# cockroachdb/pebble

Hardware: AMD Instinct MI355X
Metric: raw-block GiB/s decoded to KV arrays (device-resident), 1/2/4/8 MI355X (higher is better)
Workload: dtype u8; 1 GPU; config2: 65536 x 32 KiB row-format blocks per GPU, restart interval 16, 16 B keys / 100 B values; blocks_per_gpu=65536, input_bytes_per_gpu=2143748096, kvs_per_gpu=17760256, global_batch_blocks=65536, parallelism=shard1

## Files before the change

pebble_amd/csrc/rowblk_big.hip.h:

```cpp
#pragma once

#include "rowblk_core.hip.h"
#include "rowblk_general.hip.h"

namespace pbl {
namespace row {
namespace rowc {

#ifndef PBL_BIG_WIN
#define PBL_BIG_WIN 8
#endif
#ifndef PBL_BIG_U
#define PBL_BIG_U 8
#endif
#ifndef PBL_BIG_KEYBUF
#define PBL_BIG_KEYBUF 8192
#endif
constexpr uint32_t kBigKeySmall = PBL_BIG_KEYBUF;
constexpr int kWsBigRedo = 5;
constexpr int kWsBigPend = 6;
constexpr int kWsBigLong = 7;

__device__ __forceinline__ void big_block_publish(const Args& A, uint32_t b, const SlowState& ss) {
  const uint32_t nb = A.in.n_blocks;
  uint64_t* lb_state = reinterpret_cast<uint64_t*>(reinterpret_cast<uint8_t*>(A.out.workspace) + kWsHeader);
  const bool okk = ss.status == PBL_OK;
  const uint64_t agg[kNumComp] = {okk ? ss.nkv : 0, okk ? ss.kb : 0, okk ? ss.vb : 0, okk ? ss.nr : 0};
  lb_publish(lb_state, nb, b, agg);
  if (lane_id() == 0) {
    to_glb(A.out.blk_status)[b] = ss.status;
    to_glb(A.out.blk_kv_base)[b] = agg[0];
    to_glb(A.out.blk_key_base)[b] = agg[1];
    to_glb(A.out.blk_val_base)[b] = agg[2];
  }
}

template <bool kSpill = false>
__device__ __forceinline__ void big_block_count(const Args& A, uint32_t b, lptr<uint8_t> keybuf, uint32_t keycap,
                                                SlowState* ss, gptr<uint8_t> spill = nullptr, uint64_t spillcap = 0) {
  const uint32_t blen = A.in.block_len[b];
  const uint8_t* gblk = A.in.blocks + A.in.block_off[b];
  uint32_t roff, nres;
  const uint32_t st = init_checks(GlbBlk{to_glb(gblk), blen}, blen, A.in.flags, &roff, &nres);
  if (st != PBL_OK) {
    ss->nkv = ss->kb = ss->vb = ss->nr = 0;
    ss->status = st;
    return;
  }
  const uint64_t dummy[kNumComp] = {0, 0, 0, 0};
  slow_walk_t<GlbBlk, 1, kSpill>(GlbBlk{to_glb(gblk), blen}, blen, A.in.flags, A.in.synthetic_seq_num, keybuf, keycap,
                                  kPassCount, A.out, b, dummy, ss, spill, spillcap);
}

__global__ void __launch_bounds__(kWave) big_block_sizes_kernel(Args A) {
  __shared__ uint4 keybuf4[kBigKeySmall / 16];
  const uint32_t nb = A.in.n_blocks;
  uint32_t* hdr = reinterpret_cast<uint32_t*>(A.out.workspace);
  uint32_t* redo = reinterpret_cast<uint32_t*>(reinterpret_cast<uint8_t*>(A.out.workspace) + ws_redo_offset(nb));
  for (uint64_t base = uint64_t(blockIdx.x) * PBL_BIG_WIN; base < nb; base += uint64_t(gridDim.x) * PBL_BIG_WIN) {
    const uint64_t bl = base + lane_id();
    uint64_t big = __ballot(lane_id() < PBL_BIG_WIN && bl < nb && to_glb(A.in.block_len)[bl] > kMaxFastLen &&
                            (!A.in.block_format || to_glb(A.in.block_format)[bl] == PBL_FMT_ROW));
    while (big) {
      const uint32_t b = uint32_t(base) + uint32_t(__builtin_ctzll(big));
      big &= big - 1;
      SlowState ss;
      big_block_count(A, b, to_lds_ptr(reinterpret_cast<uint8_t*>(keybuf4)), kBigKeySmall, &ss);
      if (ss.status == PBL_UNSUPPORTED) {
        if (lane_id() == 0) to_glb(redo)[g_atomic_add(hdr + kWsBigRedo, 1u)] = b;
        continue;
      }
      big_block_publish(A, b, ss);
    }
  }
}

template <bool kList>
__device__ __forceinline__ void big_block_sizes2_body(const Args& A, uint4* keybuf4) {
  const uint32_t nb = A.in.n_blocks;
  const uint32_t* hdr = reinterpret_cast<const uint32_t*>(A.out.workspace);
  const uint32_t n = __hip_atomic_load(to_glb(hdr) + kWsBigRedo, __ATOMIC_RELAXED, __HIP_MEMORY_SCOPE_AGENT);
  const uint32_t* redo = reinterpret_cast<const uint32_t*>(reinterpret_cast<uint8_t*>(A.out.workspace) +
                                                           ws_redo_offset(nb));
  for (uint32_t i = blockIdx.x; i < n; i += gridDim.x) {
    const uint32_t b = to_glb(redo)[i];
    SlowState ss;
    big_block_count(A, b, to_lds_ptr(reinterpret_cast<uint8_t*>(keybuf4)), uint32_t(kLdsBlkBytes), &ss);
    if constexpr (kList) {
      if (ss.status == PBL_UNSUPPORTED && !((ss.kb | ss.vb) >> 32)) {
        uint32_t* lng = reinterpret_cast<uint32_t*>(reinterpret_cast<uint8_t*>(A.out.workspace) + ws_ent_offset(nb));
        if (lane_id() == 0) to_glb(lng)[g_atomic_add(const_cast<uint32_t*>(hdr) + kWsBigLong, 1u)] = b;
        continue;
      }
    }
    big_block_publish(A, b, ss);
  }
}

__global__ void __launch_bounds__(kWave) big_block_sizes2_kernel(Args A) {
  __shared__ uint4 keybuf4[kLdsBlkBytes / 16];
  big_block_sizes2_body<false>(A, keybuf4);
}

__global__ void __launch_bounds__(kWave) big_block_values_kernel(Args A) {
  __shared__ uint4 keybuf4[kLdsBlkBytes / 16];
  const uint32_t nb = A.in.n_blocks;
  const uint32_t* hdr = reinterpret_cast<const uint32_t*>(A.out.workspace);
  const uint32_t n = __hip_atomic_load(to_glb(hdr) + kWsBigPend, __ATOMIC_RELAXED, __HIP_MEMORY_SCOPE_AGENT);
  const uint32_t* pend = reinterpret_cast<const uint32_t*>(reinterpret_cast<const uint8_t*>(A.out.workspace) +
                                                           ws_pend_offset(nb));
  for (uint32_t i = blockIdx.x; i < n; i += gridDim.x) {
    const uint32_t b = to_glb(pend)[i];
    const uint32_t blen = A.in.block_len[b];
    const uint64_t bases[kNumComp] = {A.out.blk_kv_base[b], A.out.blk_key_base[b], A.out.blk_val_base[b],
                                      A.out.blk_rst_base ? A.out.blk_rst_base[b] : 0};
    SlowState ss;
    slow_walk_t<GlbBlk, PBL_BIG_U>(GlbBlk{to_glb(A.in.blocks + A.in.block_off[b]), blen}, blen, A.in.flags,
                                    A.in.synthetic_seq_num, to_lds_ptr(reinterpret_cast<uint8_t*>(keybuf4)),
                                    uint32_t(kLdsBlkBytes), kPassAll, A.out, b, bases, &ss);
  }
}

}
}
}
```

pebble_amd/csrc/rowblk_decode.hip:

```cpp
#include <algorithm>
#include <atomic>

#include "common.hip.h"
#include "colblk_block.hip.h"
#include "rowblk_core.hip.h"
#include "rowblk_general.hip.h"
#include "rowblk_big.hip.h"
#include "rowblk_pool.hip.h"
#include "rowblk_wave.hip.h"

#define PBL_COL_PIPE_BODY_ONLY
#include "colblk_pipe.hip.h"
#include "colblk_wave.hip.h"

namespace pbl {
namespace row {


__global__ void __launch_bounds__(kTPB) mixed_split_count_kernel(Args A, uint32_t* counts) {
  const uint32_t nb = A.in.n_blocks;
  const uint32_t c0 = blockIdx.x * kSplitChunk;
  uint32_t k = 0;
  for (uint32_t i = c0 + threadIdx.x; i < nb && i < c0 + kSplitChunk; i += kTPB)
    k += to_glb(A.in.block_format)[i] == PBL_FMT_ROW;
// ... 107 lines not shown
    kvb[i] += d[0];
    kb[i] += d[1];
    vb[i] += d[2];
    if (rb) rb[i] += d[3];
  }
}

}
}

namespace pbl {

namespace {
constexpr int kMaxDevices = 64;
std::atomic<int> g_cus[kMaxDevices];
std::atomic<int> g_per_cu[kMaxDevices][kKNum];
}

uint64_t persistent_grid(hipStream_t st, PersistentKernel k, const void* fn, uint64_t n_units, int* cus_out,
                         int block_threads) {
  int dev = -1;
  if (st ? hipStreamGetDevice(st, &dev) != hipSuccess : hipGetDevice(&dev) != hipSuccess) return 0;
  if (dev < 0 || dev >= kMaxDevices) return 0;
  int cus = g_cus[dev].load(std::memory_order_relaxed);
  int per_cu = g_per_cu[dev][k].load(std::memory_order_relaxed);
  if (cus <= 0 || per_cu <= 0) {
    int cur = -1;
    if (hipGetDevice(&cur) != hipSuccess) return 0;
    if (cur != dev && hipSetDevice(dev) != hipSuccess) return 0;
    const bool ok = hipDeviceGetAttribute(&cus, hipDeviceAttributeMultiprocessorCount, dev) == hipSuccess &&
                    hipOccupancyMaxActiveBlocksPerMultiprocessor(&per_cu, fn, block_threads, 0) == hipSuccess;
    if (cur != dev) (void)hipSetDevice(cur);
    if (!ok) return 0;
    cus = cus > 0 ? cus : 1;
    per_cu = per_cu > 0 ? per_cu : 1;
    g_cus[dev].store(cus, std::memory_order_relaxed);
    g_per_cu[dev][k].store(per_cu, std::memory_order_relaxed);
  }
  if (cus_out) *cus_out = cus;
  uint64_t grid = uint64_t(cus) * uint64_t(per_cu);
  if (grid > n_units) grid = n_units;
  return grid ? grid : 1;
}

}

#include "rowblk_long.hip.h"

namespace {
bool has_spill_slots(const pbl::Args& a) {
  return pbl::ws_spill_slot_bytes(a.out.workspace_bytes, a.in.n_blocks) != 0;
}

void launch_big_sizes(const pbl::Args& a, hipStream_t st, uint32_t small) {
  const uint32_t g1 = (a.in.n_blocks + PBL_BIG_WIN - 1) / PBL_BIG_WIN;
  hipLaunchKernelGGL(pbl::row::rowc::big_block_sizes_kernel, dim3(g1), dim3(pbl::kWave), 0, st, a);
  if (!has_spill_slots(a)) {
    hipLaunchKernelGGL(pbl::row::rowc::big_block_sizes2_kernel, dim3(small), dim3(pbl::kWave), 0, st, a);
    return;
  }
  hipLaunchKernelGGL(pbl::row::rowc::long_key_sizes2_kernel, dim3(small), dim3(pbl::kWave), 0, st, a);
  hipLaunchKernelGGL(pbl::row::rowc::long_key_sizes_kernel, dim3(pbl::kLongKeyWgs), dim3(pbl::kWave), 0, st, a);
}

void launch_long_values(const pbl::Args& a, hipStream_t st, uint64_t list_off, int count_word) {
  if (has_spill_slots(a))
    hipLaunchKernelGGL(pbl::row::rowc::long_key_values_kernel, dim3(pbl::kLongKeyWgs), dim3(pbl::kWave), 0, st, a,
                       list_off, count_word);
}

void launch_big_values(const pbl::Args& a, hipStream_t st, uint32_t small) {
  hipLaunchKernelGGL(pbl::row::rowc::big_block_values_kernel, dim3(small), dim3(pbl::kWave), 0, st, a);
  launch_long_values(a, st, pbl::ws_ent_offset(a.in.n_blocks), pbl::row::rowc::kWsBigLong);
}

uint64_t pool_grid(hipStream_t st, bool hide, uint32_t nb, int* cus) {
  namespace pool = pbl::row::pool;
  const void* fn = pbl::with_bool(
      hide, [](auto h) { return reinterpret_cast<const void*>(pool::rowblk_pool_kernel<decltype(h)::value>); });
  return pbl::persistent_grid(st, pbl::kKRowPool, fn, (uint64_t(nb) + pool::kNW - 1) / pool::kNW, cus, pool::kTPBP);
}

void launch_pool(const pbl::Args& a, hipStream_t st, bool hide, uint64_t grid, const uint32_t* ids) {
  namespace pool = pbl::row::pool;
  pbl::with_bool(hide, [&](auto h) {
    hipLaunchKernelGGL(pool::rowblk_pool_kernel<decltype(h)::value>, dim3(uint32_t(grid)), dim3(pool::kTPBP), 0, st, a,
                       ids);
  });
}

int launch_row_pool(const pbl::Args& a, hipStream_t st, bool values) {
  const uint32_t nb = a.in.n_blocks;
  const bool hide = (a.in.flags & PBL_ROW_HIDE_OBSOLETE) && !(a.in.flags & PBL_ROW_RAW_KEYS);
  int cus = 0;
  const uint64_t grid = pool_grid(st, hide, nb, &cus);
  if (!grid) return PBL_DEVICE_ERROR;
  const uint32_t small = uint32_t(std::min<uint64_t>(nb, uint64_t(cus > 0 ? cus : 1) * 4));
  launch_big_sizes(a, st, small);
  launch_pool(a, st, hide, grid, nullptr);
  if (values) launch_big_values(a, st, small);
  return hipGetLastError() == hipSuccess ? PBL_OK : PBL_DEVICE_ERROR;
}

int launch_mixed(const pbl_block_batch* batch, const pbl::Args& a, hipStream_t st, bool values) {
  const bool hide = (batch->flags & PBL_ROW_HIDE_OBSOLETE) != 0;
  const bool hide_rows = hide && !(batch->flags & PBL_ROW_RAW_KEYS);
  const uint32_t nb = batch->n_blocks;
  uint8_t* ws = reinterpret_cast<uint8_t*>(a.out.workspace);
  uint32_t* ids = reinterpret_cast<uint32_t*>(ws + pbl::ws_ids_offset(nb));
  uint32_t* counts = ids + nb;
  const uint32_t nch = (nb + pbl::kSplitChunk - 1) / pbl::kSplitChunk;
  hipLaunchKernelGGL(pbl::row::mixed_split_count_kernel, dim3(nch), dim3(pbl::kTPB), 0, st, a, counts);
  hipLaunchKernelGGL(pbl::row::mixed_split_scatter_kernel, dim3(nch), dim3(pbl::kTPB), 0, st, a,
                     static_cast<const uint32_t*>(counts), nch, ids);
  int cus = 0;
  const void* cfn = pbl::with_bool(
      hide, [](auto h) { return reinterpret_cast<const void*>(pbl::row::mixed_col_kernel<decltype(h)::value>); });
  const uint64_t g_c = pbl::persistent_grid(st, hide ? pbl::kKMixedColHide : pbl::kKMixedCol, cfn, nb, &cus);
  if (!g_c) return PBL_DEVICE_ERROR;
  const uint32_t small = uint32_t(std::min<uint64_t>(nb, uint64_t(cus > 0 ? cus : 1) * 4));
  const uint32_t* cids = static_cast<const uint32_t*>(ids);
  launch_big_sizes(a, st, small);
  const uint32_t g_cs = uint32_t(std::min<uint64_t>(nb, uint64_t(cus > 0 ? cus : 1) * 4 * PBL_CW_SWAVES));
  pbl::with_bool(hide, [&](auto h) {
    hipLaunchKernelGGL((pbl::col::cwave::colblk_wave_size_kernel<true, decltype(h)::value>), dim3(g_cs),
                       dim3(pbl::kWave), 0, st, a, cids);
  });
  const uint64_t g_p = pool_grid(st, hide_rows, nb, &cus);
  if (!g_p) return PBL_DEVICE_ERROR;
  launch_pool(a, st, hide_rows, g_p, cids);
#ifndef PBL_MIX_COL_WAVE
#define PBL_MIX_COL_WAVE 1
#endif
  if (!hide && PBL_MIX_COL_WAVE)
    hipLaunchKernelGGL((pbl::col::cwave::colblk_wave_emit_kernel<PBL_CW_STAGE, true>), dim3(nb), dim3(pbl::kWave), 0,
                       st, a, cids);
  else
    pbl::with_bool(hide, [&](auto h) {
      hipLaunchKernelGGL(pbl::row::mixed_col_kernel<decltype(h)::value>, dim3(uint32_t(g_c)), dim3(pbl::kTPB), 0, st,
                         a, cids);
    });
  if (values) launch_big_values(a, st, small);
  return hipGetLastError() == hipSuccess ? PBL_OK : PBL_DEVICE_ERROR;
}

int launch_row_wave(const pbl::Args& a, hipStream_t st) {
  const uint32_t nb = a.in.n_blocks;
  int dev = 0, cus = 256;
  if (hipStreamGetDevice(st, &dev) != hipSuccess ||
      hipDeviceGetAttribute(&cus, hipDeviceAttributeMultiprocessorCount, dev) != hipSuccess)
    return PBL_DEVICE_ERROR;
  namespace cw = pbl::col::cwave;
  const uint32_t nt = (nb + cw::kScanTile - 1) / cw::kScanTile;
  pbl::with_bool(has_spill_slots(a), [&](auto lk) {
    constexpr bool kLong = decltype(lk)::value;
    hipLaunchKernelGGL(pbl::row::rwave::row_wave_size_kernel<kLong>, dim3((nb + pbl::kWave - 1) / pbl::kWave),
                       dim3(pbl::kWave), 0, st, a);
    hipLaunchKernelGGL(pbl::row::rwave::row_wave_dense_kernel<kLong>, dim3(std::min<uint32_t>(nb, uint32_t(cus) * 8)),
                       dim3(pbl::kWave), 0, st, a);
    hipLaunchKernelGGL(cw::bases_scan_kernel<true>, dim3(std::min<uint32_t>(nt, uint32_t(cus) * 2)), dim3(pbl::kTPB), 0,
                       st, a);
    hipLaunchKernelGGL(pbl::row::rwave::row_wave_emit_kernel<kLong>, dim3(nb),
                       dim3(pbl::row::rwave::kRwWaves * pbl::kWave), 0, st, a);
  });
  launch_long_values(a, st, pbl::ws_pend_offset(nb), pbl::row::rowc::kWsBigPend);
  return hipGetLastError() == hipSuccess ? PBL_OK : PBL_DEVICE_ERROR;
}

int launch_row(const pbl::Args& a, hipStream_t st, bool values) {
  const uint32_t f = a.in.flags;
  if ((f & PBL_BATCH_VARLEN) && !(f & PBL_KERNEL_POOL) && pbl::row::rwave::sizes_without_keys(f))
    return launch_row_wave(a, st);
  return launch_row_pool(a, st, values);
}

bool per_block_args_ok(const pbl_block_batch* batch, const pbl_decode_out* out) {
  return batch && out && !(batch->synthetic_seq_num >> 56) &&
         out->totals && out->blk_kv_base && out->blk_key_base && out->blk_val_base && out->blk_status;
}
bool block_args_ok(const pbl_block_batch* batch, const pbl_decode_out* out) {
  return batch->blocks && batch->block_off && batch->block_len && out->workspace &&
         out->workspace_bytes >= pbl::ws_alloc_bytes(batch->n_blocks);
}
}

extern "C" {

int pbl_abi_version(void) { return PBL_ABI_VERSION; }

uint64_t pbl_workspace_bytes(uint32_t n_blocks) { return pbl::ws_alloc_bytes(n_blocks); }

uint64_t pbl_workspace_bytes_for(uint32_t n_blocks, uint32_t max_block_len) {
  const uint64_t base = pbl::ws_alloc_bytes(n_blocks);
  if (max_block_len <= pbl::row::kMaxFastLen) return base;
  return base + uint64_t(pbl::kLongKeyWgs) * ((uint64_t(max_block_len) + 15) & ~uint64_t(15));
}

int pbl_decode_batch_colblk(const pbl_block_batch* batch, pbl_decode_out* out, void* stream);

int pbl_decode_batch(const pbl_block_batch* batch, pbl_decode_out* out, void* stream) {
  if (!per_block_args_ok(batch, out)) return PBL_INVALID_ARG;
  hipStream_t st = reinterpret_cast<hipStream_t>(stream);
  if (hipMemsetAsync(out->totals, 0, sizeof(pbl_totals), st) != hipSuccess) return PBL_DEVICE_ERROR;
  if (batch->n_blocks == 0) return PBL_OK;
  if (!block_args_ok(batch, out) || !out->trailer || !out->key_off || !out->val_off || !out->key_bytes || !out->val_bytes ||
      (!out->tiering_span_id != !out->tiering_attr))
    return PBL_INVALID_ARG;
  if (!batch->block_format && batch->format != PBL_FMT_ROW) return pbl_decode_batch_colblk(batch, out, stream);
  if (hipMemsetAsync(out->workspace, 0, pbl::ws_bytes(batch->n_blocks), st) != hipSuccess)
    return PBL_DEVICE_ERROR;
  pbl::Args a;
  a.in = *batch;
  a.out = *out;
  const int rc = batch->block_format ? launch_mixed(batch, a, st, true) : launch_row(a, st, true);
  if (rc != PBL_OK || !out->tiering_span_id) return rc;
  const uint32_t g = batch->n_blocks < 8192 ? batch->n_blocks : 8192;
  hipLaunchKernelGGL(pbl::row::row_meta_zero_kernel, dim3(g), dim3(pbl::kWave), 0, st, a);
  return hipGetLastError() == hipSuccess ? PBL_OK : PBL_DEVICE_ERROR;
}

int pbl_size_batch(const pbl_block_batch* batch, pbl_decode_out* out, void* stream) {
  if (!per_block_args_ok(batch, out)) return PBL_INVALID_ARG;
  hipStream_t st = reinterpret_cast<hipStream_t>(stream);
  if (batch->n_blocks == 0) return pbl_decode_batch(batch, out, stream);
  if (!block_args_ok(batch, out)) return PBL_INVALID_ARG;
  pbl_decode_out o = *out;
  o.trailer = nullptr;
  o.kv_flags = nullptr;
  o.entry_off = nullptr;
  o.key_off = nullptr;
  o.val_off = nullptr;
  o.key_bytes = nullptr;
  o.val_bytes = nullptr;
  o.restarts = nullptr;
  o.tiering_span_id = nullptr;
  o.tiering_attr = nullptr;
  o.kv_cap = o.key_cap = o.val_cap = o.rst_cap = 0;
  if (hipMemsetAsync(o.totals, 0, sizeof(pbl_totals), st) != hipSuccess) return PBL_DEVICE_ERROR;
  if (hipMemsetAsync(o.workspace, 0, pbl::ws_bytes(batch->n_blocks), st) != hipSuccess) return PBL_DEVICE_ERROR;
  pbl::Args a;
  a.in = *batch;
  a.out = o;
  int rc = PBL_OK;
  if (!batch->block_format && batch->format != PBL_FMT_ROW) {
    rc = pbl_decode_batch_colblk(batch, &o, stream);
  } else {
    rc = batch->block_format ? launch_mixed(batch, a, st, false) : launch_row(a, st, false);
  }
  if (rc != PBL_OK) return rc;
  hipLaunchKernelGGL(pbl::row::size_fixup_kernel, dim3((batch->n_blocks + 255) / 256), dim3(256), 0, st,
                     o.blk_status, o.totals, batch->n_blocks);
  return hipGetLastError() == hipSuccess ? PBL_OK : PBL_DEVICE_ERROR;
}

size_t pbl_struct_layout(uint64_t* out, size_t cap) {
#define PBL_OFF(T, f) uint64_t(offsetof(T, f))
  const uint64_t v[] = {
      sizeof(pbl_block_batch), PBL_OFF(pbl_block_batch, blocks), PBL_OFF(pbl_block_batch, block_off),
      PBL_OFF(pbl_block_batch, block_len), PBL_OFF(pbl_block_batch, n_blocks), PBL_OFF(pbl_block_batch, format),
      PBL_OFF(pbl_block_batch, flags), PBL_OFF(pbl_block_batch, reserved), PBL_OFF(pbl_block_batch, block_format),
      PBL_OFF(pbl_block_batch, synthetic_seq_num),
      sizeof(pbl_totals), PBL_OFF(pbl_totals, n_kv), PBL_OFF(pbl_totals, key_bytes), PBL_OFF(pbl_totals, val_bytes),
      PBL_OFF(pbl_totals, n_restarts), PBL_OFF(pbl_totals, status_mask), PBL_OFF(pbl_totals, n_bad_blocks),
      PBL_OFF(pbl_totals, n_slow_blocks), PBL_OFF(pbl_totals, pad),
      sizeof(pbl_decode_out), PBL_OFF(pbl_decode_out, trailer), PBL_OFF(pbl_decode_out, kv_flags),
      PBL_OFF(pbl_decode_out, entry_off), PBL_OFF(pbl_decode_out, key_off), PBL_OFF(pbl_decode_out, val_off),
      PBL_OFF(pbl_decode_out, key_bytes), PBL_OFF(pbl_decode_out, val_bytes), PBL_OFF(pbl_decode_out, restarts),
      PBL_OFF(pbl_decode_out, blk_kv_base), PBL_OFF(pbl_decode_out, blk_key_base),
      PBL_OFF(pbl_decode_out, blk_val_base), PBL_OFF(pbl_decode_out, blk_rst_base),
      PBL_OFF(pbl_decode_out, blk_status), PBL_OFF(pbl_decode_out, totals), PBL_OFF(pbl_decode_out, kv_cap),
      PBL_OFF(pbl_decode_out, key_cap), PBL_OFF(pbl_decode_out, val_cap), PBL_OFF(pbl_decode_out, rst_cap),
      PBL_OFF(pbl_decode_out, workspace), PBL_OFF(pbl_decode_out, workspace_bytes),
      PBL_OFF(pbl_decode_out, tiering_span_id), PBL_OFF(pbl_decode_out, tiering_attr),
      sizeof(pbl_transforms), PBL_OFF(pbl_transforms, synthetic_seq_num),
      PBL_OFF(pbl_transforms, hide_obsolete_points), PBL_OFF(pbl_transforms, split), PBL_OFF(pbl_transforms, prefix),
      PBL_OFF(pbl_transforms, suffix), PBL_OFF(pbl_transforms, prefix_len), PBL_OFF(pbl_transforms, suffix_len),
      PBL_OFF(pbl_transforms, blocks),
      sizeof(pbl_footer), PBL_OFF(pbl_footer, table_format), PBL_OFF(pbl_footer, checksum_type),
      PBL_OFF(pbl_footer, metaindex_off), PBL_OFF(pbl_footer, metaindex_len), PBL_OFF(pbl_footer, index_off),
      PBL_OFF(pbl_footer, index_len), PBL_OFF(pbl_footer, footer_off), PBL_OFF(pbl_footer, footer_len),
      PBL_OFF(pbl_footer, attributes), PBL_OFF(pbl_footer, reserved),
      sizeof(pbl_index_out), PBL_OFF(pbl_index_out, handle_off), PBL_OFF(pbl_index_out, handle_len),
      PBL_OFF(pbl_index_out, props_off), PBL_OFF(pbl_index_out, props_len), PBL_OFF(pbl_index_out, blk_base),
      PBL_OFF(pbl_index_out, blk_status), PBL_OFF(pbl_index_out, cap),
      sizeof(pbl_kv_out), PBL_OFF(pbl_kv_out, key_off), PBL_OFF(pbl_kv_out, key_len), PBL_OFF(pbl_kv_out, val_off),
      PBL_OFF(pbl_kv_out, val_len), PBL_OFF(pbl_kv_out, blk_base), PBL_OFF(pbl_kv_out, blk_status),
      PBL_OFF(pbl_kv_out, cap),
      sizeof(pbl_value_out), PBL_OFF(pbl_value_out, val_off), PBL_OFF(pbl_value_out, val_bytes),
      PBL_OFF(pbl_value_out, blk_val_base), PBL_OFF(pbl_value_out, blk_status), PBL_OFF(pbl_value_out, val_cap),
      sizeof(pbl_kv), PBL_OFF(pbl_kv, user_key), PBL_OFF(pbl_kv, user_key_len), PBL_OFF(pbl_kv, trailer),
      PBL_OFF(pbl_kv, value), PBL_OFF(pbl_kv, value_len), PBL_OFF(pbl_kv, kv_flags), PBL_OFF(pbl_kv, reserved),
      sizeof(pbl_kv_meta), PBL_OFF(pbl_kv_meta, tiering_span_id), PBL_OFF(pbl_kv_meta, tiering_attribute)};
// ... 32 lines not shown
```

pebble_amd/csrc/rowblk_long.hip.h:

```cpp
#pragma once

#include "rowblk_core.hip.h"
#include "rowblk_general.hip.h"
#include "rowblk_big.hip.h"

namespace pbl {
namespace row {
namespace rowc {

struct LongSlot {
  gptr<uint8_t> p;
  uint64_t cap;
};
__device__ __forceinline__ LongSlot long_slot(const Args& A) {
  const uint32_t nb = A.in.n_blocks;
  const uint64_t cap = ws_spill_slot_bytes(A.out.workspace_bytes, nb);
  return LongSlot{to_glb(reinterpret_cast<uint8_t*>(A.out.workspace) + ws_alloc_bytes(nb) + uint64_t(blockIdx.x) * cap),
                  cap};
}

__global__ void __launch_bounds__(kWave) long_key_sizes2_kernel(Args A) {
  __shared__ uint4 keybuf4[kLdsBlkBytes / 16];
  big_block_sizes2_body<true>(A, keybuf4);
}

__global__ void __launch_bounds__(kWave) long_key_sizes_kernel(Args A) {
  __shared__ uint4 keybuf4[kLdsBlkBytes / 16];
  const uint32_t nb = A.in.n_blocks;
  const uint32_t* hdr = reinterpret_cast<const uint32_t*>(A.out.workspace);
  const uint32_t n = __hip_atomic_load(to_glb(hdr) + kWsBigLong, __ATOMIC_RELAXED, __HIP_MEMORY_SCOPE_AGENT);
  const uint32_t* lng = reinterpret_cast<const uint32_t*>(reinterpret_cast<const uint8_t*>(A.out.workspace) +
                                                          ws_ent_offset(nb));
  const LongSlot sp = long_slot(A);
  for (uint32_t i = blockIdx.x; i < n; i += gridDim.x) {
    const uint32_t b = to_glb(lng)[i];
    SlowState ss;
    big_block_count<true>(A, b, to_lds_ptr(reinterpret_cast<uint8_t*>(keybuf4)), uint32_t(kLdsBlkBytes), &ss, sp.p,
                          sp.cap);
    big_block_publish(A, b, ss);
  }
}

__global__ void __launch_bounds__(kWave) long_key_values_kernel(Args A, uint64_t list_off, int count_word) {
  __shared__ uint4 keybuf4[kLdsBlkBytes / 16];
  const pbl_decode_out& O = A.out;
  const uint32_t* hdr = reinterpret_cast<const uint32_t*>(O.workspace);
  const uint32_t n = __hip_atomic_load(to_glb(hdr) + count_word, __ATOMIC_RELAXED, __HIP_MEMORY_SCOPE_AGENT);
  const uint32_t* list = reinterpret_cast<const uint32_t*>(reinterpret_cast<const uint8_t*>(O.workspace) + list_off);
  const LongSlot sp = long_slot(A);
  for (uint32_t i = blockIdx.x; i < n; i += gridDim.x) {
    const uint32_t b = to_glb(list)[i];
    if (to_glb(O.blk_status)[b] != PBL_OK) continue;
    const uint32_t blen = to_glb(A.in.block_len)[b];
    const uint64_t bases[kNumComp] = {to_glb(O.blk_kv_base)[b], to_glb(O.blk_key_base)[b], to_glb(O.blk_val_base)[b],
                                      O.blk_rst_base ? to_glb(O.blk_rst_base)[b] : 0};
    SlowState ss;
    slow_walk_t<GlbBlk, PBL_BIG_U, true>(GlbBlk{to_glb(A.in.blocks + to_glb(A.in.block_off)[b]), blen}, blen,
                                          A.in.flags, A.in.synthetic_seq_num,
                                          to_lds_ptr(reinterpret_cast<uint8_t*>(keybuf4)), uint32_t(kLdsBlkBytes),
                                          kPassAll, O, b, bases, &ss, sp.p, sp.cap);
    if (ss.status != PBL_OK && lane_id() == 0) {
      to_glb(O.blk_status)[b] = ss.status;
      g_atomic_or(&O.totals->status_mask, 1u << ss.status);
      g_atomic_add(&O.totals->n_bad_blocks, 1u);
    }
  }
}

}
}
}
```

pebble_amd/csrc/rowblk_pool.hip.h:

```cpp
#pragma once

#include "rowblk_core.hip.h"
#include "rowblk_general.hip.h"
#include "rowblk_big.hip.h"

namespace pbl {
namespace row {
namespace pool {

#ifndef PBL_POOL_WAVES
#define PBL_POOL_WAVES 8
#endif
#ifndef PBL_POOL_STAGES
#define PBL_POOL_STAGES 3
#endif
#ifndef PBL_POOL_SLEEP
#define PBL_POOL_SLEEP 8
#endif
#ifndef PBL_POOL_PRIO
#define PBL_POOL_PRIO 2
#endif
#ifndef PBL_POOL_EARLYREL
#define PBL_POOL_EARLYREL 2
#endif
// ... 825 lines not shown
        val_store(vp, nkv, j0, B, g, vbytes);
        B = N;
      } else {
        val_store(vp, nkv, j0, B, g, vbytes);
      }
    }
  } else {
    for (uint32_t j0 = 0; j0 < nkv; j0 += 2 * S) {
      VBatch N;
      if (j0 + 2 * S < nkv) val_load(vp, g, nkv, j0 + 2 * S, N);
      val_store(vp, nkv, j0, B, g, vbytes);
      if (j0 + S >= nkv) break;
      VBatch N1;
      if (j0 + 3 * S < nkv) val_load(vp, g, nkv, j0 + 3 * S, N1);
      val_store(vp, nkv, j0 + S, B1, g, vbytes);
      B = N;
      B1 = N1;
    }
  }
  copy_long_values(vp, g, nkv, vbytes);
}

#ifndef PBL_POOL_LONGU
#define PBL_POOL_LONGU 8
#endif
constexpr int kLongU = PBL_POOL_LONGU;
__device__ __forceinline__ void copy_long_values(const uint32_t* vp, gptr<const uint8_t> g, uint32_t nkv,
                                                 gptr<uint8_t> vbytes) {
  const int l = lane_id();
  for (uint32_t j0 = 0; j0 < nkv; j0 += kWave) {
    const uint32_t j = j0 + uint32_t(l);
    const uint32_t a = j < nkv ? vp[j] : 0u, z = j < nkv ? vp[j + 1] : 0u;
    const uint32_t len = (z & 0xffffu) - (a & 0xffffu);
    for (uint64_t lm = __ballot(j < nkv && len > kWaveVal); lm; lm &= lm - 1) {
      const int sl = __builtin_ctzll(lm);
      const uint32_t ls = __shfl(a >> 16, sl, kWave), ll = __shfl(len, sl, kWave), lo = __shfl(a & 0xffffu, sl, kWave);
      for (uint32_t o0 = 16u * l; o0 < ll; o0 += 16u * kLongU * kWave) {
        u32x4 y[kLongU];
#pragma unroll
        for (int k = 0; k < kLongU; k++) {
          const uint32_t o = o0 + 16u * kWave * k, q = o < ll - 16 ? o : ll - 16;
          y[k] = *(gptr<const u32x4_ug>)(g + ls + (o < ll ? q : 0u));
        }
#pragma unroll
        for (int k = 0; k < kLongU; k++) {
          const uint32_t o = o0 + 16u * kWave * k, q = o < ll - 16 ? o : ll - 16;
          if (o < ll) st_out((gptr<u32x4_ug>)(vbytes + lo + q), u32x4_ug(y[k]));
        }
      }
    }
  }
}

template <bool kHide>
__device__ __forceinline__ uint32_t acquire(PoolLds<kHide>& L) {
  uint32_t s = 0;
  if (lane_id() == 0) {
    for (;;) {
      const uint32_t m = __hip_atomic_load(&L.free_mask, __ATOMIC_RELAXED, __HIP_MEMORY_SCOPE_WORKGROUP);
      if (m) {
        const uint32_t c = uint32_t(__builtin_ctz(m));
        const uint32_t old =
            __hip_atomic_fetch_and(&L.free_mask, ~(1u << c), __ATOMIC_ACQUIRE, __HIP_MEMORY_SCOPE_WORKGROUP);
        if (old & (1u << c)) {
          s = c;
          break;
        }
      } else {
        __builtin_amdgcn_s_sleep(PBL_POOL_SLEEP);
      }
    }
  }
  if (PBL_POOL_PRIO) __builtin_amdgcn_s_setprio(PBL_POOL_PRIO);
  return __builtin_amdgcn_readfirstlane(__shfl(s, 0, kWave));
}

template <bool kHide>
__device__ __forceinline__ int32_t try_acquire(PoolLds<kHide>& L) {
  int32_t s = -1;
  if (lane_id() == 0) {
    const uint32_t m = __hip_atomic_load(&L.free_mask, __ATOMIC_RELAXED, __HIP_MEMORY_SCOPE_WORKGROUP);
    if (m) {
      const uint32_t c = uint32_t(__builtin_ctz(m));
      const uint32_t old =
          __hip_atomic_fetch_and(&L.free_mask, ~(1u << c), __ATOMIC_ACQUIRE, __HIP_MEMORY_SCOPE_WORKGROUP);
      if (old & (1u << c)) s = int32_t(c);
    }
  }
  return __builtin_amdgcn_readfirstlane(__shfl(s, 0, kWave));
}

template <bool kHide>
__device__ __forceinline__ void release(PoolLds<kHide>& L, uint32_t s, bool drop_prio = true) {
  asm volatile("s_waitcnt lgkmcnt(0)" ::: "memory");
  wave_sync();
  if (lane_id() == 0) __hip_atomic_fetch_or(&L.free_mask, 1u << s, __ATOMIC_RELEASE, __HIP_MEMORY_SCOPE_WORKGROUP);
  if (PBL_POOL_PRIO && drop_prio) __builtin_amdgcn_s_setprio(0);
}

__device__ __forceinline__ void stage_dma(Stage& S, const uint8_t* blocks, uint64_t boff, uint32_t blen) {
  const int l = lane_id();
  const uint64_t a0 = boff & ~uint64_t(15), a1 = (boff + blen + 15) & ~uint64_t(15);
  const uint32_t n16 = uint32_t((a1 - a0) >> 4);
  const gptr<const uint8_t> base = to_glb(blocks + a0);
  for (uint32_t g0 = 0; g0 < n16; g0 += kWave) {
    if (g0 + l < n16)
      __builtin_amdgcn_global_load_lds((gptr<const void>)(base + 16ull * (g0 + l)),
                                       (lptr<void>)to_lds_ptr(reinterpret_cast<void*>(&S.x[1 + g0])), 16, 0, 0);
  }
}

__device__ __noinline__ void block_slow(Stage& S, uint8_t* keybuf, uint32_t keycap, const Args A, uint32_t b,
                                        uint64_t boff, uint32_t blen) {
  const int l = lane_id();
  const uint32_t nb = A.in.n_blocks, flags = A.in.flags;
  const pbl_decode_out& O = A.out;
  uint64_t* lb_state = reinterpret_cast<uint64_t*>(reinterpret_cast<uint8_t*>(O.workspace) + kWsHeader);
  SlowState ss;
  uint64_t dummy[kNumComp] = {0, 0, 0, 0}, excl[kNumComp];
  const uint8_t* src = reinterpret_cast<const uint8_t*>(S.x) + kPad + (boff & 15);
  bool from_lds = true;
  slow_walk(src, true, blen, flags, A.in.synthetic_seq_num, keybuf, keycap, kPassCount, O, b, dummy, &ss);
  if (ss.status == PBL_UNSUPPORTED) {
    from_lds = false;
    src = A.in.blocks + boff;
    keybuf = reinterpret_cast<uint8_t*>(S.x);
    keycap = uint32_t(kLdsBlkBytes);
    slow_walk(src, false, blen, flags, A.in.synthetic_seq_num, keybuf, keycap, kPassCount, O, b, dummy, &ss);
  }
  const bool okk = ss.status == PBL_OK;
  const uint64_t agg[kNumComp] = {okk ? ss.nkv : 0, okk ? ss.kb : 0, okk ? ss.vb : 0, okk ? ss.nr : 0};
  lookback<kLbL2, kPoolLbF>(lb_state, nb, b, agg, excl, &O.totals->status_mask);
  uint32_t st2 = ss.status;
  if (okk && overflows(O, excl, agg)) st2 = PBL_OVERFLOW;
  if (st2 == PBL_OK) slow_walk(src, from_lds, blen, flags, A.in.synthetic_seq_num, keybuf, keycap, kPassAll, O, b, excl, &ss);
  else if (l == 0 && O.key_off && excl[0] + b < O.kv_cap + nb) {
    to_glb(O.key_off)[excl[0] + b] = 0;
    to_glb(O.val_off)[excl[0] + b] = 0;
  }
  if (l == 0) write_block_meta(O, b, nb, st2, excl, agg, true);
}

__device__ __noinline__ void block_big(const Args A, uint32_t b, uint64_t boff, uint32_t blen, uint8_t* keybuf,
                                       uint32_t keycap) {
  const int l = lane_id();
  const uint32_t nb = A.in.n_blocks;
  const pbl_decode_out& O = A.out;
  uint64_t* lb_state = reinterpret_cast<uint64_t*>(reinterpret_cast<uint8_t*>(O.workspace) + kWsHeader);
  const uint32_t st0 = to_glb(O.blk_status)[b];
  const bool okk = st0 == PBL_OK;
  const uint64_t agg[kNumComp] = {okk ? to_glb(O.blk_kv_base)[b] : 0, okk ? to_glb(O.blk_key_base)[b] : 0,
                                  okk ? to_glb(O.blk_val_base)[b] : 0,
                                  okk ? uint64_t(GlbBlk{to_glb(A.in.blocks + boff), blen}.le32(blen - 4)) : 0};
  uint64_t excl[kNumComp];
  lb_resolve<kLbWin, kLbL2, kPoolLbF>(lb_state, nb, b, agg, excl, &O.totals->status_mask);
  uint32_t st2 = st0;
  if (okk && overflows(O, excl, agg)) st2 = PBL_OVERFLOW;
  if (l == 0) {
    if (st2 != PBL_OK && O.key_off && excl[0] + b < O.kv_cap + nb) {
      to_glb(O.key_off)[excl[0] + b] = 0;
      to_glb(O.val_off)[excl[0] + b] = 0;
    }
    write_block_meta(O, b, nb, st2, excl, agg, true);
  }
  if (st2 == PBL_OK) {
    SlowState ss;
    slow_walk_t<GlbBlk, PBL_BIG_U>(GlbBlk{to_glb(A.in.blocks + boff), blen}, blen, A.in.flags,
                                    A.in.synthetic_seq_num, to_lds_ptr(keybuf), keycap, kPassAll, O, b, excl, &ss);
    if (ss.status == PBL_UNSUPPORTED && l == 0) {
      uint32_t* hdr = reinterpret_cast<uint32_t*>(O.workspace);
      uint32_t* pend = reinterpret_cast<uint32_t*>(reinterpret_cast<uint8_t*>(O.workspace) + ws_pend_offset(nb));
      to_glb(pend)[g_atomic_add(hdr + rowc::kWsBigPend, 1u)] = b;
    } else if (ss.status != PBL_OK && l == 0) {
      to_glb(O.blk_status)[b] = ss.status;
      g_atomic_or(&O.totals->status_mask, 1u << ss.status);
      g_atomic_add(&O.totals->n_bad_blocks, 1u);
    }
  }
}

struct Pend {
  uint64_t boff;
  uint32_t b, status, nkv, tkb, tvb, nres, roff, blen;
  bool live;
};

template <bool kHide>
__device__ __forceinline__ Pend block_front(PoolLds<kHide>& L, uint32_t s, uint32_t b, uint64_t boff, uint32_t blen,
                                            bool staged, Slot<kHide>& W, const Args& A) {
  Stage& S = L.st[s];
  const int l = lane_id();
  const uint32_t nb = A.in.n_blocks, flags = A.in.flags;
  const bool vprefix = (flags & PBL_ROW_VALUE_PREFIX) && !(flags & PBL_ROW_RAW_KEYS);
  uint64_t* lb_state = reinterpret_cast<uint64_t*>(reinterpret_cast<uint8_t*>(A.out.workspace) + kWsHeader);
  constexpr uint32_t kKv = uint32_t(Slot<kHide>::kKv);
  Pend P;
  P.b = b;
  P.boff = boff;
  P.blen = blen;
  P.live = false;
  P.nkv = P.tkb = P.tvb = P.nres = P.roff = 0;
  P.status = PBL_OK;

  if (blen > kMaxFastLen) {
    release(L, s);
    block_big(A, b, boff, blen, reinterpret_cast<uint8_t*>(&W), uint32_t(sizeof(W)));
    return P;
  }
  PSTAMP(A, b, 1, l == 0);
  if (!staged) stage_dma(S, A.in.blocks, boff, blen);
  asm volatile("s_waitcnt vmcnt(0)" ::: "memory");
  wave_sync();
  PSTAMP(A, b, 2, l == 0);
  const View V = lds_view(S.x, uint32_t(kPad + (boff & 15)));
  uint32_t roff, nres;
  uint32_t status = init_checks(LdsBlk{V}, blen, flags, &roff, &nres);
  bool slow = status == PBL_OK && nres > kKv;
  uint32_t nkv = 0, tkb = 0, tvb = 0;
  bool published = false, released = false;
  if (status == PBL_OK && !slow && roff > 0) {
    const uint32_t R = (nres + kWave - 1) / kWave;
    const uint32_t r0 = min(uint32_t(l) * R, nres), r1 = min(r0 + R, nres);
    PAcc acc{0, 0, 0, 0};
    bool ok = true, bad = false, vbad = false, over = false;
    PRun RB;
    RB.n = 0;
    RB.pos = RB.e0 = RB.prev_kl = RB.prev_kind = RB.rw = 0;
    const bool single = R == 1;
    walk_runs<kHide>(V, r0, r1, nres, roff, flags, vprefix, single, RB, acc, ok, bad, vbad, over);
    const uint32_t ic = dpp_incl_scan(acc.cnt), ik = dpp_incl_scan(acc.kb), iv = dpp_incl_scan(acc.vb);
    const uint32_t ie = kHide ? dpp_incl_scan(acc.ne) : ic;
    nkv = last_lane(ic);
    tkb = last_lane(ik);
    tvb = last_lane(iv);
    const uint32_t nent = kHide ? last_lane(ie) : nkv;
    if (__ballot(bad)) status = PBL_CORRUPT_BOUNDS;
    else if (__ballot(!ok) || nent > kKv) slow = true;
    else if (__ballot(vbad)) status = PBL_CORRUPT_BOUNDS;
    if (status == PBL_OK && !slow) {
      const uint64_t agg[kNumComp] = {nkv, tkb, tvb, nres};
      lb_publish(lb_state, nb, b, agg);
      published = true;
      PSTAMP(A, b, 3, l == 0);
      if (kEarlyRel && single && !vprefix && !__ballot(over)) {
        release(L, s, kEarlyRel != 2);
        released = true;
        PSTAMP(A, b, 9, l == 0);
      }
      MState M{ie - (kHide ? acc.ne : acc.cnt), ic - acc.cnt, iv - acc.vb, 0, 0, 0};
      meta_runs<kHide>(W, V, r0, r1, nres, roff, flags, vprefix, single, over, RB, M);
      if (l < 5) W.vp[nkv + l] = tvb;
      PSTAMP(A, b, 4, l == 0);
    }
  }
  if (status == PBL_OK && slow) {
    block_slow(S, reinterpret_cast<uint8_t*>(W.m0), uint32_t(sizeof(W.m0)), A, b, boff, blen);
    release(L, s);
    PSTAMP(A, b, 9, l == 0);
    return P;
// ... 247 lines not shown
```

Baseline: 1661 GiB/s.

## Fold workspace/totals zeroing into prepare kernel and inline big-block redo into pool

Replaces the host-side hipMemsetAsync of totals and the full workspace with zeroing done inside a new row_prepare_kernel, which clears only the look-back records, prefix and L2 entries it needs while also scanning for big blocks. Big blocks that need a larger key buffer are no longer queued to separate sizes2/values kernels. They are marked in blk_status and recounted or re-walked inside the pool kernel, using a borrowed LDS stage buffer. This removes a memset over the large workspace plus two extra kernel launches, at the cost of more complex stage acquire/release logic inside the pool kernel. It also relies on the prepare kernel's zeroing being complete, since the pool path no longer memsets.

```diff
diff --git a/pebble_amd/csrc/rowblk_big.hip.h b/pebble_amd/csrc/rowblk_big.hip.h
--- a/pebble_amd/csrc/rowblk_big.hip.h
+++ b/pebble_amd/csrc/rowblk_big.hip.h
@@ -20,6 +20,7 @@
 constexpr int kWsBigRedo = 5;
 constexpr int kWsBigPend = 6;
 constexpr int kWsBigLong = 7;
+constexpr uint32_t kBigRedo = 0x80000000u | PBL_UNSUPPORTED;
 
 __device__ __forceinline__ void big_block_publish(const Args& A, uint32_t b, const SlowState& ss) {
   const uint32_t nb = A.in.n_blocks;
@@ -52,22 +53,39 @@
                                   kPassCount, A.out, b, dummy, ss, spill, spillcap);
 }
 
-__global__ void __launch_bounds__(kWave) big_block_sizes_kernel(Args A) {
+__global__ void __launch_bounds__(kWave) row_prepare_kernel(Args A) {
   __shared__ uint4 keybuf4[kBigKeySmall / 16];
+  static_assert(sizeof(pbl_totals) % 8 == 0 && kWsHeader / 8 <= kWave && sizeof(pbl_totals) / 8 <= kWave, "one store per lane");
   const uint32_t nb = A.in.n_blocks;
-  uint32_t* hdr = reinterpret_cast<uint32_t*>(A.out.workspace);
-  uint32_t* redo = reinterpret_cast<uint32_t*>(reinterpret_cast<uint8_t*>(A.out.workspace) + ws_redo_offset(nb));
+  const uint32_t l = lane_id();
+  uint64_t* ws = reinterpret_cast<uint64_t*>(A.out.workspace);
+  const LbPtrs P(ws + kWsHeader / 8, nb);
+  if (blockIdx.x == 0) {
+    if (l < kWsHeader / 8) st_agent(ws + l, 0);
+    if (l < sizeof(pbl_totals) / 8) st_agent(reinterpret_cast<uint64_t*>(A.out.totals) + l, 0);
+  }
   for (uint64_t base = uint64_t(blockIdx.x) * PBL_BIG_WIN; base < nb; base += uint64_t(gridDim.x) * PBL_BIG_WIN) {
-    const uint64_t bl = base + lane_id();
-    uint64_t big = __ballot(lane_id() < PBL_BIG_WIN && bl < nb && to_glb(A.in.block_len)[bl] > kMaxFastLen &&
+    const uint32_t n = nb - base < PBL_BIG_WIN ? uint32_t(nb - base) : uint32_t(PBL_BIG_WIN);
+    for (uint32_t i = l; i < 2 * n; i += kWave) st_agent(P.rec + 2 * base + i, 0);
+    for (uint32_t i = l; i < 2 * kNumComp * PBL_BIG_WIN; i += kWave) {
+      const uint32_t a = i / PBL_BIG_WIN, j = i % PBL_BIG_WIN;
+      if (j < n) st_agent(P.pfx + uint64_t(a) * nb + base + j, 0);
+    }
+    for (uint64_t c = (base + kL2Chunk - 1) / kL2Chunk + l; c * kL2Chunk < base + n; c += kWave) {
+      st_agent(P.l2 + 2 * c, 0);
+      st_agent(P.l2 + 2 * c + 1, 0);
+    }
+    const uint64_t bl = base + l;
+    uint64_t big = __ballot(l < PBL_BIG_WIN && bl < nb && to_glb(A.in.block_len)[bl] > kMaxFastLen &&
                             (!A.in.block_format || to_glb(A.in.block_format)[bl] == PBL_FMT_ROW));
+    if (big) asm volatile("s_waitcnt vmcnt(0)" ::: "memory");
     while (big) {
       const uint32_t b = uint32_t(base) + uint32_t(__builtin_ctzll(big));
       big &= big - 1;
       SlowState ss;
       big_block_count(A, b, to_lds_ptr(reinterpret_cast<uint8_t*>(keybuf4)), kBigKeySmall, &ss);
       if (ss.status == PBL_UNSUPPORTED) {
-        if (lane_id() == 0) to_glb(redo)[g_atomic_add(hdr + kWsBigRedo, 1u)] = b;
+        if (l == 0) to_glb(A.out.blk_status)[b] = kBigRedo;
         continue;
       }
       big_block_publish(A, b, ss);
@@ -75,52 +93,6 @@
   }
 }
 
-template <bool kList>
-__device__ __forceinline__ void big_block_sizes2_body(const Args& A, uint4* keybuf4) {
-  const uint32_t nb = A.in.n_blocks;
-  const uint32_t* hdr = reinterpret_cast<const uint32_t*>(A.out.workspace);
-  const uint32_t n = __hip_atomic_load(to_glb(hdr) + kWsBigRedo, __ATOMIC_RELAXED, __HIP_MEMORY_SCOPE_AGENT);
-  const uint32_t* redo = reinterpret_cast<const uint32_t*>(reinterpret_cast<uint8_t*>(A.out.workspace) +
-                                                           ws_redo_offset(nb));
-  for (uint32_t i = blockIdx.x; i < n; i += gridDim.x) {
-    const uint32_t b = to_glb(redo)[i];
-    SlowState ss;
-    big_block_count(A, b, to_lds_ptr(reinterpret_cast<uint8_t*>(keybuf4)), uint32_t(kLdsBlkBytes), &ss);
-    if constexpr (kList) {
-      if (ss.status == PBL_UNSUPPORTED && !((ss.kb | ss.vb) >> 32)) {
-        uint32_t* lng = reinterpret_cast<uint32_t*>(reinterpret_cast<uint8_t*>(A.out.workspace) + ws_ent_offset(nb));
-        if (lane_id() == 0) to_glb(lng)[g_atomic_add(const_cast<uint32_t*>(hdr) + kWsBigLong, 1u)] = b;
-        continue;
-      }
-    }
-    big_block_publish(A, b, ss);
-  }
-}
-
-__global__ void __launch_bounds__(kWave) big_block_sizes2_kernel(Args A) {
-  __shared__ uint4 keybuf4[kLdsBlkBytes / 16];
-  big_block_sizes2_body<false>(A, keybuf4);
-}
-
-__global__ void __launch_bounds__(kWave) big_block_values_kernel(Args A) {
-  __shared__ uint4 keybuf4[kLdsBlkBytes / 16];
-  const uint32_t nb = A.in.n_blocks;
-  const uint32_t* hdr = reinterpret_cast<const uint32_t*>(A.out.workspace);
-  const uint32_t n = __hip_atomic_load(to_glb(hdr) + kWsBigPend, __ATOMIC_RELAXED, __HIP_MEMORY_SCOPE_AGENT);
-  const uint32_t* pend = reinterpret_cast<const uint32_t*>(reinterpret_cast<const uint8_t*>(A.out.workspace) +
-                                                           ws_pend_offset(nb));
-  for (uint32_t i = blockIdx.x; i < n; i += gridDim.x) {
-    const uint32_t b = to_glb(pend)[i];
-    const uint32_t blen = A.in.block_len[b];
-    const uint64_t bases[kNumComp] = {A.out.blk_kv_base[b], A.out.blk_key_base[b], A.out.blk_val_base[b],
-                                      A.out.blk_rst_base ? A.out.blk_rst_base[b] : 0};
-    SlowState ss;
-    slow_walk_t<GlbBlk, PBL_BIG_U>(GlbBlk{to_glb(A.in.blocks + A.in.block_off[b]), blen}, blen, A.in.flags,
-                                    A.in.synthetic_seq_num, to_lds_ptr(reinterpret_cast<uint8_t*>(keybuf4)),
-                                    uint32_t(kLdsBlkBytes), kPassAll, A.out, b, bases, &ss);
-  }
-}
-
 }
 }
 }
diff --git a/pebble_amd/csrc/rowblk_decode.hip b/pebble_amd/csrc/rowblk_decode.hip
--- a/pebble_amd/csrc/rowblk_decode.hip
+++ b/pebble_amd/csrc/rowblk_decode.hip
@@ -183,13 +183,13 @@
   return pbl::ws_spill_slot_bytes(a.out.workspace_bytes, a.in.n_blocks) != 0;
 }
 
-void launch_big_sizes(const pbl::Args& a, hipStream_t st, uint32_t small) {
+void launch_prepare(const pbl::Args& a, hipStream_t st) {
   const uint32_t g1 = (a.in.n_blocks + PBL_BIG_WIN - 1) / PBL_BIG_WIN;
-  hipLaunchKernelGGL(pbl::row::rowc::big_block_sizes_kernel, dim3(g1), dim3(pbl::kWave), 0, st, a);
-  if (!has_spill_slots(a)) {
-    hipLaunchKernelGGL(pbl::row::rowc::big_block_sizes2_kernel, dim3(small), dim3(pbl::kWave), 0, st, a);
-    return;
-  }
+  hipLaunchKernelGGL(pbl::row::rowc::row_prepare_kernel, dim3(g1), dim3(pbl::kWave), 0, st, a);
+}
+
+void launch_long_sizes(const pbl::Args& a, hipStream_t st, uint32_t small) {
+  if (!has_spill_slots(a)) return;
   hipLaunchKernelGGL(pbl::row::rowc::long_key_sizes2_kernel, dim3(small), dim3(pbl::kWave), 0, st, a);
   hipLaunchKernelGGL(pbl::row::rowc::long_key_sizes_kernel, dim3(pbl::kLongKeyWgs), dim3(pbl::kWave), 0, st, a);
 }
@@ -198,11 +198,6 @@
   if (has_spill_slots(a))
     hipLaunchKernelGGL(pbl::row::rowc::long_key_values_kernel, dim3(pbl::kLongKeyWgs), dim3(pbl::kWave), 0, st, a,
                        list_off, count_word);
-}
-
-void launch_big_values(const pbl::Args& a, hipStream_t st, uint32_t small) {
-  hipLaunchKernelGGL(pbl::row::rowc::big_block_values_kernel, dim3(small), dim3(pbl::kWave), 0, st, a);
-  launch_long_values(a, st, pbl::ws_ent_offset(a.in.n_blocks), pbl::row::rowc::kWsBigLong);
 }
 
 uint64_t pool_grid(hipStream_t st, bool hide, uint32_t nb, int* cus) {
@@ -227,9 +222,10 @@
   const uint64_t grid = pool_grid(st, hide, nb, &cus);
   if (!grid) return PBL_DEVICE_ERROR;
   const uint32_t small = uint32_t(std::min<uint64_t>(nb, uint64_t(cus > 0 ? cus : 1) * 4));
-  launch_big_sizes(a, st, small);
+  launch_prepare(a, st);
+  launch_long_sizes(a, st, small);
   launch_pool(a, st, hide, grid, nullptr);
-  if (values) launch_big_values(a, st, small);
+  if (values) launch_long_values(a, st, pbl::ws_ent_offset(nb), pbl::row::rowc::kWsBigLong);
   return hipGetLastError() == hipSuccess ? PBL_OK : PBL_DEVICE_ERROR;
 }
 
@@ -241,6 +237,7 @@
   uint32_t* ids = reinterpret_cast<uint32_t*>(ws + pbl::ws_ids_offset(nb));
   uint32_t* counts = ids + nb;
   const uint32_t nch = (nb + pbl::kSplitChunk - 1) / pbl::kSplitChunk;
+  launch_prepare(a, st);
   hipLaunchKernelGGL(pbl::row::mixed_split_count_kernel, dim3(nch), dim3(pbl::kTPB), 0, st, a, counts);
   hipLaunchKernelGGL(pbl::row::mixed_split_scatter_kernel, dim3(nch), dim3(pbl::kTPB), 0, st, a,
                      static_cast<const uint32_t*>(counts), nch, ids);
@@ -251,7 +248,7 @@
   if (!g_c) return PBL_DEVICE_ERROR;
   const uint32_t small = uint32_t(std::min<uint64_t>(nb, uint64_t(cus > 0 ? cus : 1) * 4));
   const uint32_t* cids = static_cast<const uint32_t*>(ids);
-  launch_big_sizes(a, st, small);
+  launch_long_sizes(a, st, small);
   const uint32_t g_cs = uint32_t(std::min<uint64_t>(nb, uint64_t(cus > 0 ? cus : 1) * 4 * PBL_CW_SWAVES));
   pbl::with_bool(hide, [&](auto h) {
     hipLaunchKernelGGL((pbl::col::cwave::colblk_wave_size_kernel<true, decltype(h)::value>), dim3(g_cs),
@@ -271,7 +268,7 @@
       hipLaunchKernelGGL(pbl::row::mixed_col_kernel<decltype(h)::value>, dim3(uint32_t(g_c)), dim3(pbl::kTPB), 0, st,
                          a, cids);
     });
-  if (values) launch_big_values(a, st, small);
+  if (values) launch_long_values(a, st, pbl::ws_ent_offset(nb), pbl::row::rowc::kWsBigLong);
   return hipGetLastError() == hipSuccess ? PBL_OK : PBL_DEVICE_ERROR;
 }
 
@@ -298,11 +295,15 @@
   return hipGetLastError() == hipSuccess ? PBL_OK : PBL_DEVICE_ERROR;
 }
 
+bool row_wave_path(uint32_t f) {
+  return (f & PBL_BATCH_VARLEN) && !(f & PBL_KERNEL_POOL) && pbl::row::rwave::sizes_without_keys(f);
+}
 int launch_row(const pbl::Args& a, hipStream_t st, bool values) {
-  const uint32_t f = a.in.flags;
-  if ((f & PBL_BATCH_VARLEN) && !(f & PBL_KERNEL_POOL) && pbl::row::rwave::sizes_without_keys(f))
-    return launch_row_wave(a, st);
-  return launch_row_pool(a, st, values);
+  return row_wave_path(a.in.flags) ? launch_row_wave(a, st) : launch_row_pool(a, st, values);
+}
+
+bool pool_path(const pbl_block_batch* batch) {
+  return batch->block_format || (batch->format == PBL_FMT_ROW && !row_wave_path(batch->flags));
 }
 
 bool per_block_args_ok(const pbl_block_batch* batch, const pbl_decode_out* out) {
@@ -332,13 +333,15 @@
 int pbl_decode_batch(const pbl_block_batch* batch, pbl_decode_out* out, void* stream) {
   if (!per_block_args_ok(batch, out)) return PBL_INVALID_ARG;
   hipStream_t st = reinterpret_cast<hipStream_t>(stream);
-  if (hipMemsetAsync(out->totals, 0, sizeof(pbl_totals), st) != hipSuccess) return PBL_DEVICE_ERROR;
+  const bool args_ok = batch->n_blocks == 0 ||
+                       (block_args_ok(batch, out) && out->trailer && out->key_off && out->val_off && out->key_bytes &&
+                        out->val_bytes && (!out->tiering_span_id == !out->tiering_attr));
+  const bool prepared = batch->n_blocks != 0 && args_ok && pool_path(batch);
+  if (!prepared && hipMemsetAsync(out->totals, 0, sizeof(pbl_totals), st) != hipSuccess) return PBL_DEVICE_ERROR;
   if (batch->n_blocks == 0) return PBL_OK;
-  if (!block_args_ok(batch, out) || !out->trailer || !out->key_off || !out->val_off || !out->key_bytes || !out->val_bytes ||
-      (!out->tiering_span_id != !out->tiering_attr))
-    return PBL_INVALID_ARG;
+  if (!args_ok) return PBL_INVALID_ARG;
   if (!batch->block_format && batch->format != PBL_FMT_ROW) return pbl_decode_batch_colblk(batch, out, stream);
-  if (hipMemsetAsync(out->workspace, 0, pbl::ws_bytes(batch->n_blocks), st) != hipSuccess)
+  if (!prepared && hipMemsetAsync(out->workspace, 0, pbl::ws_bytes(batch->n_blocks), st) != hipSuccess)
     return PBL_DEVICE_ERROR;
   pbl::Args a;
   a.in = *batch;
@@ -367,8 +370,10 @@
   o.tiering_span_id = nullptr;
   o.tiering_attr = nullptr;
   o.kv_cap = o.key_cap = o.val_cap = o.rst_cap = 0;
-  if (hipMemsetAsync(o.totals, 0, sizeof(pbl_totals), st) != hipSuccess) return PBL_DEVICE_ERROR;
-  if (hipMemsetAsync(o.workspace, 0, pbl::ws_bytes(batch->n_blocks), st) != hipSuccess) return PBL_DEVICE_ERROR;
+  if (!pool_path(batch)) {
+    if (hipMemsetAsync(o.totals, 0, sizeof(pbl_totals), st) != hipSuccess) return PBL_DEVICE_ERROR;
+    if (hipMemsetAsync(o.workspace, 0, pbl::ws_bytes(batch->n_blocks), st) != hipSuccess) return PBL_DEVICE_ERROR;
+  }
   pbl::Args a;
   a.in = *batch;
   a.out = o;
diff --git a/pebble_amd/csrc/rowblk_long.hip.h b/pebble_amd/csrc/rowblk_long.hip.h
--- a/pebble_amd/csrc/rowblk_long.hip.h
+++ b/pebble_amd/csrc/rowblk_long.hip.h
@@ -21,7 +21,26 @@
 
 __global__ void __launch_bounds__(kWave) long_key_sizes2_kernel(Args A) {
   __shared__ uint4 keybuf4[kLdsBlkBytes / 16];
-  big_block_sizes2_body<true>(A, keybuf4);
+  const uint32_t nb = A.in.n_blocks;
+  uint32_t* hdr = reinterpret_cast<uint32_t*>(A.out.workspace);
+  uint32_t* lng = reinterpret_cast<uint32_t*>(reinterpret_cast<uint8_t*>(A.out.workspace) + ws_ent_offset(nb));
+  for (uint64_t base = uint64_t(blockIdx.x) * kWave; base < nb; base += uint64_t(gridDim.x) * kWave) {
+    const uint64_t bl = base + lane_id();
+    uint64_t redo = __ballot(bl < nb && to_glb(A.in.block_len)[bl] > kMaxFastLen &&
+                             (!A.in.block_format || to_glb(A.in.block_format)[bl] == PBL_FMT_ROW) &&
+                             to_glb(A.out.blk_status)[bl] == kBigRedo);
+    while (redo) {
+      const uint32_t b = uint32_t(base) + uint32_t(__builtin_ctzll(redo));
+      redo &= redo - 1;
+      SlowState ss;
+      big_block_count(A, b, to_lds_ptr(reinterpret_cast<uint8_t*>(keybuf4)), uint32_t(kLdsBlkBytes), &ss);
+      if (ss.status == PBL_UNSUPPORTED && !((ss.kb | ss.vb) >> 32)) {
+        if (lane_id() == 0) to_glb(lng)[g_atomic_add(hdr + kWsBigLong, 1u)] = b;
+        continue;
+      }
+      big_block_publish(A, b, ss);
+    }
+  }
 }
 
 __global__ void __launch_bounds__(kWave) long_key_sizes_kernel(Args A) {
diff --git a/pebble_amd/csrc/rowblk_pool.hip.h b/pebble_amd/csrc/rowblk_pool.hip.h
--- a/pebble_amd/csrc/rowblk_pool.hip.h
+++ b/pebble_amd/csrc/rowblk_pool.hip.h
@@ -901,16 +901,16 @@
   }
 }
 
-template <bool kHide>
-__device__ __forceinline__ uint32_t acquire(PoolLds<kHide>& L) {
+template <class M>
+__device__ __forceinline__ uint32_t acquire_stage(M* free_mask) {
   uint32_t s = 0;
   if (lane_id() == 0) {
     for (;;) {
-      const uint32_t m = __hip_atomic_load(&L.free_mask, __ATOMIC_RELAXED, __HIP_MEMORY_SCOPE_WORKGROUP);
+      const uint32_t m = __hip_atomic_load(free_mask, __ATOMIC_RELAXED, __HIP_MEMORY_SCOPE_WORKGROUP);
       if (m) {
         const uint32_t c = uint32_t(__builtin_ctz(m));
         const uint32_t old =
-            __hip_atomic_fetch_and(&L.free_mask, ~(1u << c), __ATOMIC_ACQUIRE, __HIP_MEMORY_SCOPE_WORKGROUP);
+            __hip_atomic_fetch_and(free_mask, ~(1u << c), __ATOMIC_ACQUIRE, __HIP_MEMORY_SCOPE_WORKGROUP);
         if (old & (1u << c)) {
           s = c;
           break;
@@ -922,6 +922,10 @@
   }
   if (PBL_POOL_PRIO) __builtin_amdgcn_s_setprio(PBL_POOL_PRIO);
   return __builtin_amdgcn_readfirstlane(__shfl(s, 0, kWave));
+}
+template <bool kHide>
+__device__ __forceinline__ uint32_t acquire(PoolLds<kHide>& L) {
+  return acquire_stage(&L.free_mask);
 }
 
 template <bool kHide>
@@ -939,12 +943,16 @@
   return __builtin_amdgcn_readfirstlane(__shfl(s, 0, kWave));
 }
 
-template <bool kHide>
-__device__ __forceinline__ void release(PoolLds<kHide>& L, uint32_t s, bool drop_prio = true) {
+template <class M>
+__device__ __forceinline__ void release_stage(M* free_mask, uint32_t s, bool drop_prio = true) {
   asm volatile("s_waitcnt lgkmcnt(0)" ::: "memory");
   wave_sync();
-  if (lane_id() == 0) __hip_atomic_fetch_or(&L.free_mask, 1u << s, __ATOMIC_RELEASE, __HIP_MEMORY_SCOPE_WORKGROUP);
+  if (lane_id() == 0) __hip_atomic_fetch_or(free_mask, 1u << s, __ATOMIC_RELEASE, __HIP_MEMORY_SCOPE_WORKGROUP);
   if (PBL_POOL_PRIO && drop_prio) __builtin_amdgcn_s_setprio(0);
+}
+template <bool kHide>
+__device__ __forceinline__ void release(PoolLds<kHide>& L, uint32_t s, bool drop_prio = true) {
+  release_stage(&L.free_mask, s, drop_prio);
 }
 
 __device__ __forceinline__ void stage_dma(Stage& S, const uint8_t* blocks, uint64_t boff, uint32_t blen) {
@@ -991,16 +999,34 @@
 }
 
 __device__ __noinline__ void block_big(const Args A, uint32_t b, uint64_t boff, uint32_t blen, uint8_t* keybuf,
-                                       uint32_t keycap) {
+                                       uint32_t keycap, Stage* stages, uint32_t* free_mask, uint32_t s) {
   const int l = lane_id();
   const uint32_t nb = A.in.n_blocks;
   const pbl_decode_out& O = A.out;
+  const lptr<uint32_t> fm = to_lds_ptr(free_mask);
   uint64_t* lb_state = reinterpret_cast<uint64_t*>(reinterpret_cast<uint8_t*>(O.workspace) + kWsHeader);
-  const uint32_t st0 = to_glb(O.blk_status)[b];
+  uint32_t st0 = to_glb(O.blk_status)[b];
+  uint64_t agg[kNumComp];
+  if (st0 == rowc::kBigRedo) {
+    SlowState ss;
+    rowc::big_block_count(A, b, to_lds_ptr(reinterpret_cast<uint8_t*>(stages[s].x)), uint32_t(kLdsBlkBytes), &ss);
+    rowc::big_block_publish(A, b, ss);
+    release_stage(fm, s);
+    st0 = ss.status;
+    const bool ok2 = st0 == PBL_OK;
+    agg[0] = ok2 ? ss.nkv : 0;
+    agg[1] = ok2 ? ss.kb : 0;
+    agg[2] = ok2 ? ss.vb : 0;
+    agg[3] = ok2 ? ss.nr : 0;
+  } else {
+    release_stage(fm, s);
+    const bool ok1 = st0 == PBL_OK;
+    agg[0] = ok1 ? to_glb(O.blk_kv_base)[b] : 0;
+    agg[1] = ok1 ? to_glb(O.blk_key_base)[b] : 0;
+    agg[2] = ok1 ? to_glb(O.blk_val_base)[b] : 0;
+    agg[3] = ok1 ? uint64_t(GlbBlk{to_glb(A.in.blocks + boff), blen}.le32(blen - 4)) : 0;
+  }
   const bool okk = st0 == PBL_OK;
-  const uint64_t agg[kNumComp] = {okk ? to_glb(O.blk_kv_base)[b] : 0, okk ? to_glb(O.blk_key_base)[b] : 0,
-                                  okk ? to_glb(O.blk_val_base)[b] : 0,
-                                  okk ? uint64_t(GlbBlk{to_glb(A.in.blocks + boff), blen}.le32(blen - 4)) : 0};
   uint64_t excl[kNumComp];
   lb_resolve<kLbWin, kLbL2, kPoolLbF>(lb_state, nb, b, agg, excl, &O.totals->status_mask);
   uint32_t st2 = st0;
@@ -1013,14 +1039,21 @@
     write_block_meta(O, b, nb, st2, excl, agg, true);
   }
   if (st2 == PBL_OK) {
+    lptr<uint8_t> kb = to_lds_ptr(keybuf);
+    bool staged = false;
+    uint32_t s2 = 0;
     SlowState ss;
-    slow_walk_t<GlbBlk, PBL_BIG_U>(GlbBlk{to_glb(A.in.blocks + boff), blen}, blen, A.in.flags,
-                                    A.in.synthetic_seq_num, to_lds_ptr(keybuf), keycap, kPassAll, O, b, excl, &ss);
-    if (ss.status == PBL_UNSUPPORTED && l == 0) {
-      uint32_t* hdr = reinterpret_cast<uint32_t*>(O.workspace);
-      uint32_t* pend = reinterpret_cast<uint32_t*>(reinterpret_cast<uint8_t*>(O.workspace) + ws_pend_offset(nb));
-      to_glb(pend)[g_atomic_add(hdr + rowc::kWsBigPend, 1u)] = b;
-    } else if (ss.status != PBL_OK && l == 0) {
+    for (;;) {
+      slow_walk_t<GlbBlk, PBL_BIG_U>(GlbBlk{to_glb(A.in.blocks + boff), blen}, blen, A.in.flags,
+                                      A.in.synthetic_seq_num, kb, keycap, kPassAll, O, b, excl, &ss);
+      if (staged || ss.status != PBL_UNSUPPORTED) break;
+      s2 = acquire_stage(fm);
+      staged = true;
+      kb = to_lds_ptr(reinterpret_cast<uint8_t*>(stages[s2].x));
+      keycap = uint32_t(kLdsBlkBytes);
+    }
+    if (staged) release_stage(fm, s2);
+    if (!staged && ss.status != PBL_OK && l == 0) {
       to_glb(O.blk_status)[b] = ss.status;
       g_atomic_or(&O.totals->status_mask, 1u << ss.status);
       g_atomic_add(&O.totals->n_bad_blocks, 1u);
@@ -1052,8 +1085,7 @@
   P.status = PBL_OK;
 
   if (blen > kMaxFastLen) {
-    release(L, s);
-    block_big(A, b, boff, blen, reinterpret_cast<uint8_t*>(&W), uint32_t(sizeof(W)));
+    block_big(A, b, boff, blen, reinterpret_cast<uint8_t*>(&W), uint32_t(sizeof(W)), L.st, &L.free_mask, s);
     return P;
   }
   PSTAMP(A, b, 1, l == 0);
```

Measured after the change: 1686 GiB/s (median of 6 runs). 1.5% higher.
